# lukecq1231/nats

Measured on NVIDIA H100. Metric: decoder tokens/sec (dim=1000, src=400, |V|=30k) @1/2/4/8 H100 vs Theano CPU, higher is better.
Workload: dtype f32

## Files before the change

nats_b200/csrc/gemm.cu:

```cuda
#include "gemm.cuh"

namespace nats {

namespace {

constexpr int kPad = 4;

template <int BX, int BK, int NT, int PT>
__device__ __forceinline__ void load_kcontig(const float* __restrict__ src, int ld, int x0, int X, int k0,
                                             int kend, bool vec, int tid, float4 (&r)[PT]) {
#pragma unroll
    for (int i = 0; i < PT; ++i) {
        const int v = tid + i * NT;
        float4 val = make_float4(0.f, 0.f, 0.f, 0.f);
        if (v < BX * BK / 4) {
            const int x = v / (BK / 4), kq = (v % (BK / 4)) * 4;
            const int gx = x0 + x, gk = k0 + kq;
            if (gx < X && gk < kend) {
                const float* p = src + (long long)gx * ld + gk;
                if (vec && gk + 3 < kend) {
                    val = __ldg(reinterpret_cast<const float4*>(p));
                } else {
                    val.x = __ldg(p);
                    if (gk + 1 < kend) val.y = __ldg(p + 1);
// ... 210 lines not shown
    else if (ta && !tb) le = launch_pdl(sgemm_kernel<BM, BN, BK, TM, TN, true, false>, grid, block, 0, st, grp);
    else le = launch_pdl(sgemm_kernel<BM, BN, BK, TM, TN, true, true>, grid, block, 0, st, grp);
    NATS_CUDA_OK(le);
    return 0;
}

__global__ void reduce_splits_kernel(const float* __restrict__ part, int nsplit, long long strideP, int M, int N,
                                     int ldp, float* __restrict__ out, int ldo, const float* __restrict__ bias,
                                     int accumulate) {
    pdl_trigger();
    pdl_wait();
    const long long total = (long long)M * N;
    for (long long i = blockIdx.x * (long long)blockDim.x + threadIdx.x; i < total;
         i += (long long)gridDim.x * blockDim.x) {
        const int m = (int)(i / N), n = (int)(i % N);
        float s = sum_strided(part + (long long)m * ldp + n, strideP, nsplit);
        if (bias) s += __ldg(bias + n);
        float* o = out + (long long)m * ldo + n;
        if (accumulate) s += *o;
        *o = s;
    }
}

}

static int g_use_tc = 2;
void gemm_set_tensor_cores(int on) { g_use_tc = on; }
int gemm_get_tensor_cores() { return g_use_tc; }

static bool tc_eligible(const GemmProblem* probs, int count) {
    if (!g_use_tc) return false;
    for (int i = 0; i < count; ++i) {
        const int big = probs[i].M > probs[i].N ? probs[i].M : probs[i].N;
        if (big < 64 || probs[i].K < 32) return false;
    }
    return true;
}


int gemm_launch(cudaStream_t st, const GemmProblem* probs, int count, bool transA, bool transB, int cfg) {
    NATS_REQUIRE(count >= 1 && count <= kGemmMaxGroup, "gemm group size");
    if (tc_eligible(probs, count)) {
        if (g_use_tc >= 2 && tma_gemm_eligible(probs, count)) return tma_gemm_launch(st, probs, count, transA, transB);
        return tc_gemm_launch(st, probs, count, transA, transB);
    }
    GemmGroup grp;
    memset(&grp, 0, sizeof(grp));
    grp.count = count;
    int z = 0, maxM = 0, minN = 1 << 30;
    for (int i = 0; i < count; ++i) {
        grp.p[i] = probs[i];
        NATS_REQUIRE(probs[i].splitk >= 1 && probs[i].splitk <= kGemmMaxSplit && probs[i].batch >= 1, "gemm split/batch");
        NATS_REQUIRE(probs[i].splitk == 1 || !probs[i].accumulate, "split-K cannot accumulate in place");
        NATS_REQUIRE(probs[i].kchunk % 16 == 0 && probs[i].kchunk > 0, "kchunk");
        grp.zstart[i] = z;
        z += probs[i].batch * probs[i].splitk;
        maxM = max(maxM, probs[i].M);
        minN = min(minN, probs[i].N);
    }
    grp.zstart[count] = z;
    for (int i = count; i < kGemmMaxGroup; ++i) grp.zstart[i + 1] = z;
    if (maxM == 0) return 0;
    if (cfg == GEMM_CFG_AUTO) {
        if (maxM <= 32) cfg = GEMM_CFG_SMALLM;
        else if (maxM >= 512 && minN >= 512) cfg = GEMM_CFG_BIG;
        else cfg = GEMM_CFG_MID;
    }
    switch (cfg) {
        case GEMM_CFG_BIG: return launch_cfg<128, 128, 8, 8, 8>(st, grp, transA, transB);
        case GEMM_CFG_MID: return launch_cfg<64, 64, 16, 4, 4>(st, grp, transA, transB);
        case GEMM_CFG_SMALLM: return launch_cfg<32, 128, 16, 4, 4>(st, grp, transA, transB);
        default: break;
    }
    set_error("gemm_launch: bad cfg %d", cfg);
    return 2;
}

int gemm_step_cfg(int M) { return M <= 32 ? GEMM_CFG_SMALLM : GEMM_CFG_MID; }

int gemm_pick_split(const nats_ctx* ctx, int M, int N, int K, int groups) {
    int tiles;
    if (g_use_tc && (M >= 128 || N >= 128) && K >= 32) {
        const int a = M > N ? M : N, b = M > N ? N : M;
        const int bn = b <= 32 ? 32 : 64;
        tiles = cdiv(a, 128) * cdiv(b, bn);
    } else {
        const int bm = (M <= 32) ? 32 : 64, bn = (M <= 32) ? 128 : 64;
        tiles = cdiv(N, bn) * cdiv(M, bm);
    }
    tiles *= (groups > 0 ? groups : 1);
    int s = ctx->num_sms / (tiles > 0 ? tiles : 1);
    s = min(s, K / 64);
    s = min(s, kGemmMaxSplit);
    s = max(s, 1);
    const int chunk = ((cdiv(K, s) + 31) / 32) * 32;
    return max(cdiv(K, chunk), 1);
}

int reduce_splits(cudaStream_t st, const float* part, int nsplit, long long strideP, int M, int N, int ldp,
                  float* out, int ldo, const float* bias, int accumulate) {
    const long long total = (long long)M * N;
    if (total == 0) return 0;
    const int block = 256;
    long long gl = (total + block - 1) / block;
    if (gl > 132LL * 16) gl = 132LL * 16;
    const int grid = (int)gl;
    ProfScope ps(st, K_REDUCE_SPLITS, 0.0, 4.0 * total * (nsplit + 1));
    NATS_CUDA_OK(launch_pdl(reduce_splits_kernel, dim3(grid), dim3(block), 0, st, part, nsplit, strideP, M, N, ldp, out, ldo, bias,
                            accumulate));
    return 0;
}

int gemm_auto(const nats_ctx* ctx, cudaStream_t st, GemmProblem p, bool transA, bool transB, float* scratch,
              long long scratch_floats) {
    if (p.M == 0 || p.N == 0) return 0;
    const bool tc = tc_eligible(&p, 1);
    int cfg = GEMM_CFG_AUTO;
    long long tiles;
    if (tc) {
        const int a = p.M > p.N ? p.M : p.N, b = p.M > p.N ? p.N : p.M;
        const bool swapped = p.M < 128 && p.N > p.M;
        const int nb = swapped ? p.M : p.N, ma = swapped ? p.N : p.M;
        (void)a; (void)b;
        const int bn = nb <= 32 ? 32 : 64;
        tiles = (long long)cdiv(ma, 128) * cdiv(nb, bn) * p.batch;
    } else {
        int bm, bn;
        if (p.M <= 32) { cfg = GEMM_CFG_SMALLM; bm = 32; bn = 128; }
        else if (p.M >= 512 && p.N >= 512) { cfg = GEMM_CFG_BIG; bm = 128; bn = 128; }
        else { cfg = GEMM_CFG_MID; bm = 64; bn = 64; }
        tiles = (long long)cdiv(p.M, bm) * cdiv(p.N, bn) * p.batch;
    }
    int splits = 1;
    if (tc && p.batch == 1 && tiles >= ctx->num_sms && p.K >= 4096 && scratch != nullptr) {
        double best = 1e30;
        for (int s2 = 1; s2 <= 4; ++s2) {
            if ((long long)s2 * p.M * p.N > scratch_floats) break;
            const long long waves = (tiles * s2 + ctx->num_sms - 1) / ctx->num_sms;
            double t = (double)waves * ((double)p.K / s2 / 32.0 * 0.75 + 3.0);
            if (s2 > 1) t += (double)(s2 + 1) * p.M * p.N * 4.0 / 5.0e6;
            if (t < best) { best = t; splits = s2; }
        }
    } else if (p.batch == 1 && tiles < ctx->num_sms && p.K >= 256 && scratch != nullptr) {
        long long want = ((tc ? 1LL : 2LL) * ctx->num_sms + tiles - 1) / tiles;
        if (want > p.K / 128) want = p.K / 128;
        splits = (int)want;
        splits = min(splits, kGemmMaxSplit);
        while (splits > 1 && (long long)splits * p.M * p.N > scratch_floats) --splits;
        if (splits < 1) splits = 1;
    }
    if (splits == 1) return gemm_launch(st, &p, 1, transA, transB, cfg);
    GemmProblem q = p;
    q.C = scratch; q.ldc = p.N; q.bias = nullptr; q.accumulate = 0;
    gemm_set_split(q, splits, (long long)p.M * p.N);
    NATS_TRY(gemm_launch(st, &q, 1, transA, transB, cfg));
    return reduce_splits(st, scratch, splits, (long long)p.M * p.N, p.M, p.N, p.N, p.C, p.ldc, p.bias, p.accumulate);
}

}
```

nats_b200/csrc/tc_common.cuh:

```cuda
#pragma once
#include <cuda.h>

#include "common.cuh"

namespace nats {

bool tma_available();
int tma_map_tile3d(const float* ptr, long long d0, long long d1, long long d2, long long stride1, long long stride2, int b0,
                   int b1, int b2, CUtensorMap* out);

namespace tc {

__device__ __forceinline__ uint32_t smem_u32(const void* p) { return static_cast<uint32_t>(__cvta_generic_to_shared(p)); }
__device__ __forceinline__ void mbar_init(uint64_t* bar, uint32_t count) {
    asm volatile("mbarrier.init.shared::cta.b64 [%0], %1;" ::"r"(smem_u32(bar)), "r"(count) : "memory");
}
__device__ __forceinline__ void mbar_arrive(uint64_t* bar) {
    asm volatile("mbarrier.arrive.shared::cta.b64 _, [%0];" ::"r"(smem_u32(bar)) : "memory");
}
__device__ __forceinline__ void mbar_expect_tx(uint64_t* bar, uint32_t bytes) {
    asm volatile("mbarrier.arrive.expect_tx.shared::cta.b64 _, [%0], %1;" ::"r"(smem_u32(bar)), "r"(bytes) : "memory");
}
__device__ __forceinline__ void mbar_wait(uint64_t* bar, uint32_t parity) {
    uint32_t ok;
    const uint32_t addr = smem_u32(bar);
    do {
        asm volatile(
            "{\n\t.reg .pred p;\n\t"
            "mbarrier.try_wait.parity.shared::cta.b64 p, [%1], %2;\n\t"
            "selp.u32 %0, 1, 0, p;\n\t}"
            : "=r"(ok)
            : "r"(addr), "r"(parity)
            : "memory");
    } while (!ok);
}
__device__ __forceinline__ void tma_load_3d(uint32_t dst, const CUtensorMap* map, uint64_t* bar, int c0, int c1, int c2) {
    asm volatile(
        "cp.async.bulk.tensor.3d.shared::cluster.global.tile.mbarrier::complete_tx::bytes [%0], [%1, {%3, %4, %5}], [%2];"
        ::"r"(dst), "l"(reinterpret_cast<uint64_t>(map)), "r"(smem_u32(bar)), "r"(c0), "r"(c1), "r"(c2)
        : "memory");
}
__device__ __forceinline__ uint64_t desc_sw128(uint32_t saddr) {
    return (uint64_t)((saddr & 0x3FFFF) >> 4) | ((uint64_t)1 << 16) | ((uint64_t)(1024 >> 4) << 32) | ((uint64_t)1 << 62);
}
__device__ __forceinline__ void wgmma_fence() { asm volatile("wgmma.fence.sync.aligned;" ::: "memory"); }
__device__ __forceinline__ void wgmma_commit() { asm volatile("wgmma.commit_group.sync.aligned;" ::: "memory"); }
template <int N>
__device__ __forceinline__ void wgmma_wait() { asm volatile("wgmma.wait_group.sync.aligned %0;" ::"n"(N) : "memory"); }
template <int R>
__device__ __forceinline__ void reg_fence(float (&d)[R]) {
#pragma unroll
    for (int i = 0; i < R; ++i) asm volatile("" : "+f"(d[i])::"memory");
}

__device__ __forceinline__ void wgmma_ss_n32(float (&d)[16], uint64_t da, uint64_t db) {
    asm volatile(
        "{\n\t.reg .pred p;\n\tsetp.ne.b32 p, %18, 0;\n\t"
        "wgmma.mma_async.sync.aligned.m64n32k8.f32.tf32.tf32 {%0,%1,%2,%3,%4,%5,%6,%7,%8,%9,%10,%11,%12,%13,%14,%15}, %16, %17, p, 1, 1;\n\t}"
        : "+f"(d[0]), "+f"(d[1]), "+f"(d[2]), "+f"(d[3]), "+f"(d[4]), "+f"(d[5]), "+f"(d[6]), "+f"(d[7]), "+f"(d[8]), "+f"(d[9]), "+f"(d[10]), "+f"(d[11]), "+f"(d[12]), "+f"(d[13]), "+f"(d[14]), "+f"(d[15])
        : "l"(da), "l"(db), "r"(1));
}
__device__ __forceinline__ void wgmma_ss_n64(float (&d)[32], uint64_t da, uint64_t db) {
    asm volatile(
        "{\n\t.reg .pred p;\n\tsetp.ne.b32 p, %34, 0;\n\t"
        "wgmma.mma_async.sync.aligned.m64n64k8.f32.tf32.tf32 {%0,%1,%2,%3,%4,%5,%6,%7,%8,%9,%10,%11,%12,%13,%14,%15,%16,%17,%18,%19,%20,%21,%22,%23,%24,%25,%26,%27,%28,%29,%30,%31}, %32, %33, p, 1, 1;\n\t}"
        : "+f"(d[0]), "+f"(d[1]), "+f"(d[2]), "+f"(d[3]), "+f"(d[4]), "+f"(d[5]), "+f"(d[6]), "+f"(d[7]), "+f"(d[8]), "+f"(d[9]), "+f"(d[10]), "+f"(d[11]), "+f"(d[12]), "+f"(d[13]), "+f"(d[14]), "+f"(d[15]), "+f"(d[16]), "+f"(d[17]), "+f"(d[18]), "+f"(d[19]), "+f"(d[20]), "+f"(d[21]), "+f"(d[22]), "+f"(d[23]), "+f"(d[24]), "+f"(d[25]), "+f"(d[26]), "+f"(d[27]), "+f"(d[28]), "+f"(d[29]), "+f"(d[30]), "+f"(d[31])
        : "l"(da), "l"(db), "r"(1));
}
__device__ __forceinline__ void wgmma_ss_n128(float (&d)[64], uint64_t da, uint64_t db) {
    asm volatile(
        "{\n\t.reg .pred p;\n\tsetp.ne.b32 p, %66, 0;\n\t"
        "wgmma.mma_async.sync.aligned.m64n128k8.f32.tf32.tf32 {%0,%1,%2,%3,%4,%5,%6,%7,%8,%9,%10,%11,%12,%13,%14,%15,%16,%17,%18,%19,%20,%21,%22,%23,%24,%25,%26,%27,%28,%29,%30,%31,%32,%33,%34,%35,%36,%37,%38,%39,%40,%41,%42,%43,%44,%45,%46,%47,%48,%49,%50,%51,%52,%53,%54,%55,%56,%57,%58,%59,%60,%61,%62,%63}, %64, %65, p, 1, 1;\n\t}"
        : "+f"(d[0]), "+f"(d[1]), "+f"(d[2]), "+f"(d[3]), "+f"(d[4]), "+f"(d[5]), "+f"(d[6]), "+f"(d[7]), "+f"(d[8]), "+f"(d[9]), "+f"(d[10]), "+f"(d[11]), "+f"(d[12]), "+f"(d[13]), "+f"(d[14]), "+f"(d[15]), "+f"(d[16]), "+f"(d[17]), "+f"(d[18]), "+f"(d[19]), "+f"(d[20]), "+f"(d[21]), "+f"(d[22]), "+f"(d[23]), "+f"(d[24]), "+f"(d[25]), "+f"(d[26]), "+f"(d[27]), "+f"(d[28]), "+f"(d[29]), "+f"(d[30]), "+f"(d[31]), "+f"(d[32]), "+f"(d[33]), "+f"(d[34]), "+f"(d[35]), "+f"(d[36]), "+f"(d[37]), "+f"(d[38]), "+f"(d[39]), "+f"(d[40]), "+f"(d[41]), "+f"(d[42]), "+f"(d[43]), "+f"(d[44]), "+f"(d[45]), "+f"(d[46]), "+f"(d[47]), "+f"(d[48]), "+f"(d[49]), "+f"(d[50]), "+f"(d[51]), "+f"(d[52]), "+f"(d[53]), "+f"(d[54]), "+f"(d[55]), "+f"(d[56]), "+f"(d[57]), "+f"(d[58]), "+f"(d[59]), "+f"(d[60]), "+f"(d[61]), "+f"(d[62]), "+f"(d[63])
        : "l"(da), "l"(db), "r"(1));
}
__device__ __forceinline__ void wgmma_rs_n32(float (&d)[16], const uint32_t (&a)[4], uint64_t db) {
    asm volatile(
        "{\n\t.reg .pred p;\n\tsetp.ne.b32 p, %21, 0;\n\t"
        "wgmma.mma_async.sync.aligned.m64n32k8.f32.tf32.tf32 {%0,%1,%2,%3,%4,%5,%6,%7,%8,%9,%10,%11,%12,%13,%14,%15}, {%16,%17,%18,%19}, %20, p, 1, 1;\n\t}"
        : "+f"(d[0]), "+f"(d[1]), "+f"(d[2]), "+f"(d[3]), "+f"(d[4]), "+f"(d[5]), "+f"(d[6]), "+f"(d[7]), "+f"(d[8]), "+f"(d[9]), "+f"(d[10]), "+f"(d[11]), "+f"(d[12]), "+f"(d[13]), "+f"(d[14]), "+f"(d[15])
        : "r"(a[0]), "r"(a[1]), "r"(a[2]), "r"(a[3]), "l"(db), "r"(1));
}
__device__ __forceinline__ void wgmma_rs_n64(float (&d)[32], const uint32_t (&a)[4], uint64_t db) {
    asm volatile(
        "{\n\t.reg .pred p;\n\tsetp.ne.b32 p, %37, 0;\n\t"
        "wgmma.mma_async.sync.aligned.m64n64k8.f32.tf32.tf32 {%0,%1,%2,%3,%4,%5,%6,%7,%8,%9,%10,%11,%12,%13,%14,%15,%16,%17,%18,%19,%20,%21,%22,%23,%24,%25,%26,%27,%28,%29,%30,%31}, {%32,%33,%34,%35}, %36, p, 1, 1;\n\t}"
        : "+f"(d[0]), "+f"(d[1]), "+f"(d[2]), "+f"(d[3]), "+f"(d[4]), "+f"(d[5]), "+f"(d[6]), "+f"(d[7]), "+f"(d[8]), "+f"(d[9]), "+f"(d[10]), "+f"(d[11]), "+f"(d[12]), "+f"(d[13]), "+f"(d[14]), "+f"(d[15]), "+f"(d[16]), "+f"(d[17]), "+f"(d[18]), "+f"(d[19]), "+f"(d[20]), "+f"(d[21]), "+f"(d[22]), "+f"(d[23]), "+f"(d[24]), "+f"(d[25]), "+f"(d[26]), "+f"(d[27]), "+f"(d[28]), "+f"(d[29]), "+f"(d[30]), "+f"(d[31])
        : "r"(a[0]), "r"(a[1]), "r"(a[2]), "r"(a[3]), "l"(db), "r"(1));
}

__device__ __forceinline__ float to_tf32(float x) {
    uint32_t r;
    asm("cvt.rna.tf32.f32 %0, %1;" : "=r"(r) : "f"(x));
    return __uint_as_float(r);
}
__device__ __forceinline__ void st_shared_v4(uint32_t addr, float4 v) {
    asm volatile("st.shared.v4.f32 [%0], {%1,%2,%3,%4};" ::"r"(addr), "f"(v.x), "f"(v.y), "f"(v.z), "f"(v.w) : "memory");
}
__device__ __forceinline__ float resid(float x) { return x - __uint_as_float(__float_as_uint(x) & 0xFFFFE000u); }

template <int R>
__device__ __forceinline__ void gemm_epilogue(const float (&acc0)[R], const float (&acc1)[R], const float (&accx)[R], float* C,
                                              long long c_rs, long long c_cs, int Ma, int Nb, int rb, int cb,
                                              const float* bias_a, const float* bias_n, bool accumulate) {
#pragma unroll
    for (int h = 0; h < 2; ++h) {
        const int i_row = rb + 8 * h;
        if (i_row >= Ma) continue;
        const float ba = bias_a ? __ldg(bias_a + i_row) : 0.f;
        float* crow = C + (long long)i_row * c_rs;
#pragma unroll
        for (int j = 0; j < R / 4; ++j) {
#pragma unroll
            for (int e = 0; e < 2; ++e) {
                const int idx = 4 * j + 2 * h + e;
                const int col = cb + 8 * j + e;
                if (col < Nb) {
                    float o = (acc0[idx] + acc1[idx]) + accx[idx] + ba;
                    if (bias_n) o += __ldg(bias_n + col);
                    float* cp = crow + (long long)col * c_cs;
                    if (accumulate) o += *cp;
                    *cp = o;
                }
            }
        }
    }
}

__device__ __forceinline__ void named_bar_sync(int id, int nthreads) {
    asm volatile("bar.sync %0, %1;" ::"r"(id), "r"(nthreads) : "memory");
}

}
}
```

nats_b200/csrc/tma_gemm.cu:

```cuda
#include <cuda.h>

#include <unordered_map>

#include "gemm.cuh"
#include "ops.cuh"
#include "tc_common.cuh"

namespace nats {

namespace {

typedef CUresult (*EncodeTiledFn)(CUtensorMap*, CUtensorMapDataType, cuuint32_t, void*, const cuuint64_t*,
                                  const cuuint64_t*, const cuuint32_t*, const cuuint32_t*, CUtensorMapInterleave,
                                  CUtensorMapSwizzle, CUtensorMapL2promotion, CUtensorMapFloatOOBfill);
EncodeTiledFn g_encode = nullptr;

struct MapKey {
    const void* ptr; long long inner, outer, ld, batch, bstride; int box_outer; int mn;
    bool operator==(const MapKey& o) const {
        return ptr == o.ptr && inner == o.inner && outer == o.outer && ld == o.ld && batch == o.batch &&
               bstride == o.bstride && box_outer == o.box_outer && mn == o.mn;
    }
};
struct MapKeyHash {
    size_t operator()(const MapKey& k) const {
        size_t h = std::hash<const void*>()(k.ptr);
        auto mix = [&](long long v) { h ^= std::hash<long long>()(v) + 0x9e3779b97f4a7c15ull + (h << 6) + (h >> 2); };
        mix(k.inner); mix(k.outer); mix(k.ld); mix(k.batch); mix(k.bstride); mix(k.box_outer); mix(k.mn);
        return h;
    }
};
std::unordered_map<MapKey, CUtensorMap, MapKeyHash> g_maps;


constexpr int kThreads = 256;
constexpr int kBlockK = 32;
constexpr int kNR = 3;
constexpr int kMaxGroup = 2;

struct TmaProblem {
    float* C;
    const float* bias;
    int Ma, Nb, K;
    long long c_rs, c_cs;
    int batch;
    long long sC;
    int splitk, kchunk;
    long long strideP;
    int accumulate;
    int bias_on_a;
};
struct alignas(64) TmaGroup {
    CUtensorMap mapA[kMaxGroup];
    CUtensorMap mapB[kMaxGroup];
    TmaProblem p[kMaxGroup];
    int zstart[kMaxGroup + 1];
    int count;
};

using namespace tc;

template <int ROWS, bool MN>
__device__ __forceinline__ float raw_at(uint32_t raw, int r, int k) {
    float v;
    asm volatile("ld.shared.f32 %0, [%1];" : "=f"(v) : "r"(raw + 4u * (uint32_t)(MN ? k * ROWS + r : r * 32 + k)));
    return v;
}

template <int ROWS, bool MN>
__device__ __forceinline__ void split_tile(uint32_t raw, uint32_t hi_base, uint32_t lo_base, int klim, int tid) {
    constexpr int kChunks = ROWS * 8;
#pragma unroll
    for (int i = 0; i < (kChunks + kThreads - 1) / kThreads; ++i) {
        const int q = tid + i * kThreads;
        if (q < kChunks) {
            int r, c;
            float4 v;
            if (!MN) {
                r = q >> 3; c = q & 7;
                asm volatile("ld.shared.v4.f32 {%0,%1,%2,%3}, [%4];" : "=f"(v.x), "=f"(v.y), "=f"(v.z), "=f"(v.w)
                             : "r"(raw + 4u * (uint32_t)(r * 32 + 4 * c)));
            } else {
                r = q % ROWS; c = q / ROWS;
                v.x = raw_at<ROWS, true>(raw, r, 4 * c); v.y = raw_at<ROWS, true>(raw, r, 4 * c + 1);
                v.z = raw_at<ROWS, true>(raw, r, 4 * c + 2); v.w = raw_at<ROWS, true>(raw, r, 4 * c + 3);
            }
            if (4 * c >= klim) v.x = 0.f;
            if (4 * c + 1 >= klim) v.y = 0.f;
            if (4 * c + 2 >= klim) v.z = 0.f;
            if (4 * c + 3 >= klim) v.w = 0.f;
            float4 hi, lo;
            hi.x = to_tf32(v.x); hi.y = to_tf32(v.y); hi.z = to_tf32(v.z); hi.w = to_tf32(v.w);
            lo.x = to_tf32(v.x - hi.x); lo.y = to_tf32(v.y - hi.y); lo.z = to_tf32(v.z - hi.z); lo.w = to_tf32(v.w - hi.w);
            const uint32_t off = (uint32_t)(r * 128 + ((c ^ (r & 7)) << 4));
            st_shared_v4(hi_base + off, hi);
            st_shared_v4(lo_base + off, lo);
        }
    }
}

template <int BN>
__device__ __forceinline__ void mma_ss(float (&d)[BN / 2], uint64_t da, uint64_t db) {
    if constexpr (BN == 32) wgmma_ss_n32(d, da, db);
    else wgmma_ss_n64(d, da, db);
}
template <int BN>
__device__ __forceinline__ void mma_rs(float (&d)[BN / 2], const uint32_t (&a)[4], uint64_t db) {
    if constexpr (BN == 32) wgmma_rs_n32(d, a, db);
    else wgmma_rs_n64(d, a, db);
}

template <int BN, bool A_MN, bool B_MN, bool A_REG>
__global__ void __launch_bounds__(kThreads, 1) tma_gemm_kernel(const __grid_constant__ TmaGroup grp) {
    constexpr uint32_t kARaw = 128 * 128, kBRaw = BN * 128;
    constexpr uint32_t kRawStage = kARaw + kBRaw;
    constexpr uint32_t kAHalf = A_REG ? 0 : 128 * 128;
    constexpr uint32_t kSplitStage = 2 * kAHalf + 2 * kBRaw;
    constexpr uint32_t kSplitBase = kNR * kRawStage;
    constexpr int R = BN / 2;
    static_assert(BN == 32 || BN == 64, "BN");

    extern __shared__ __align__(1024) unsigned char smem[];
    __shared__ __align__(8) uint64_t full[kNR];

    int z = blockIdx.z, g = 0;
    if (grp.count > 1 && z >= grp.zstart[1]) g = 1;
    const TmaProblem& P = grp.p[g];
    const CUtensorMap* mapA = &grp.mapA[g];
    const CUtensorMap* mapB = &grp.mapB[g];
    z -= grp.zstart[g];
    const int split = z % P.splitk, batch = z / P.splitk;
    const int m0 = blockIdx.x * 128, n0 = blockIdx.y * BN;
    if (m0 >= P.Ma || n0 >= P.Nb) return;

    const int kbeg = split * P.kchunk;
    const int kend = min(P.K, kbeg + P.kchunk);
    const int nkb = (kend > kbeg) ? (kend - kbeg + kBlockK - 1) / kBlockK : 0;
    const int tid = threadIdx.x, warp = tid >> 5, lane = tid & 31, wg = tid >> 7;
    const uint32_t smem_base = (smem_u32(smem) + 1023u) & ~1023u;

    if (tid == 0) {
        asm volatile("prefetch.tensormap [%0];" ::"l"(mapA) : "memory");
        asm volatile("prefetch.tensormap [%0];" ::"l"(mapB) : "memory");
        for (int s = 0; s < kNR; ++s) mbar_init(&full[s], 1);
        asm volatile("fence.mbarrier_init.release.cluster;" ::: "memory");
    }
    __syncthreads();
    pdl_trigger();
    pdl_wait();

    auto issue = [&](int kb) {
        const int s = kb % kNR;
        const uint32_t raw = smem_base + (uint32_t)s * kRawStage;
        const int k0 = kbeg + kb * kBlockK;
        mbar_expect_tx(&full[s], kRawStage);
        if (A_MN) tma_load_3d(raw, mapA, &full[s], m0, k0, batch);
        else tma_load_3d(raw, mapA, &full[s], k0, m0, batch);
        if (B_MN) tma_load_3d(raw + kARaw, mapB, &full[s], n0, k0, batch);
        else tma_load_3d(raw + kARaw, mapB, &full[s], k0, n0, batch);
    };
    auto split_stage = [&](int kb) {
        mbar_wait(&full[kb % kNR], (uint32_t)((kb / kNR) & 1));
        const uint32_t raw = smem_base + (uint32_t)(kb % kNR) * kRawStage;
        const uint32_t sp = smem_base + kSplitBase + (uint32_t)(kb & 1) * kSplitStage;
        const int klim = kend - (kbeg + kb * kBlockK);
        if (!A_REG) split_tile<128, A_MN>(raw, sp, sp + kAHalf, klim, tid);
        split_tile<BN, B_MN>(raw + kARaw, sp + 2 * kAHalf, sp + 2 * kAHalf + kBRaw, klim, tid);
    };

    float acc0[R], acc1[R], accx[R];
#pragma unroll
    for (int i = 0; i < R; ++i) { acc0[i] = 0.f; acc1[i] = 0.f; accx[i] = 0.f; }
    const int r0 = 64 * wg + 16 * (warp & 3) + (lane >> 2);
    const int q = lane & 3;

    if (nkb > 0) {
        if (tid == 0)
            for (int kb = 0; kb < min(nkb, kNR); ++kb) issue(kb);
        split_stage(0);
    }
    asm volatile("fence.proxy.async.shared::cta;" ::: "memory");
    __syncthreads();
    for (int kb = 0; kb < nkb; ++kb) {
        const uint32_t sp = smem_base + kSplitBase + (uint32_t)(kb & 1) * kSplitStage;
        const uint64_t b_hi = desc_sw128(sp + 2 * kAHalf), b_lo = desc_sw128(sp + 2 * kAHalf + kBRaw);
        if constexpr (A_REG) {
            const uint32_t raw = smem_base + (uint32_t)(kb % kNR) * kRawStage;
            const int klim = kend - (kbeg + kb * kBlockK);
            uint32_t ahi[4][4], alo[4][4];
#pragma unroll
            for (int kk = 0; kk < 4; ++kk) {
#pragma unroll
                for (int f = 0; f < 4; ++f) {
                    const int r = r0 + 8 * (f & 1), k = 8 * kk + q + 4 * (f >> 1);
                    const float x = k < klim ? raw_at<128, A_MN>(raw, r, k) : 0.f;
                    const float h = to_tf32(x);
                    ahi[kk][f] = __float_as_uint(h);
                    alo[kk][f] = __float_as_uint(to_tf32(x - h));
                }
            }
            wgmma_fence();
#pragma unroll
            for (int kk = 0; kk < 4; ++kk) {
                mma_rs<BN>(accx, alo[kk], b_hi + 2 * kk);
                mma_rs<BN>(accx, ahi[kk], b_lo + 2 * kk);
                mma_rs<BN>((kk & 1) ? acc1 : acc0, ahi[kk], b_hi + 2 * kk);
            }
        } else {
            const uint64_t a_hi = desc_sw128(sp + (uint32_t)wg * 8192u), a_lo = desc_sw128(sp + kAHalf + (uint32_t)wg * 8192u);
            wgmma_fence();
#pragma unroll
            for (int kk = 0; kk < 4; ++kk) {
                mma_ss<BN>(accx, a_lo + 2 * kk, b_hi + 2 * kk);
                mma_ss<BN>(accx, a_hi + 2 * kk, b_lo + 2 * kk);
                mma_ss<BN>((kk & 1) ? acc1 : acc0, a_hi + 2 * kk, b_hi + 2 * kk);
            }
        }
        wgmma_commit();
        if (kb + 1 < nkb) split_stage(kb + 1);
        wgmma_wait<0>();
        reg_fence(acc0); reg_fence(acc1); reg_fence(accx);
        asm volatile("fence.proxy.async.shared::cta;" ::: "memory");
        __syncthreads();
        if (tid == 0 && kb + kNR < nkb) issue(kb + kNR);
    }

    const bool add_bias = (P.bias != nullptr) && (split == 0);
    gemm_epilogue(acc0, acc1, accx, P.C + (long long)batch * P.sC + (long long)split * P.strideP, P.c_rs, P.c_cs, P.Ma, P.Nb,
                  m0 + r0, n0 + 2 * q, (add_bias && P.bias_on_a) ? P.bias : nullptr,
                  (add_bias && !P.bias_on_a) ? P.bias : nullptr, P.accumulate != 0);
}

template <int BN, bool A_REG>
constexpr size_t smem_bytes() {
    return (size_t)kNR * (128 * 128 + BN * 128) + 2 * (size_t)(2 * (A_REG ? 0 : 128 * 128) + 2 * BN * 128) + 1024;
}

template <int BN, bool A_REG>
int set_attrs() {
    const int sm = (int)smem_bytes<BN, A_REG>();
    NATS_CUDA_OK(cudaFuncSetAttribute(tma_gemm_kernel<BN, false, false, A_REG>, cudaFuncAttributeMaxDynamicSharedMemorySize, sm));
    NATS_CUDA_OK(cudaFuncSetAttribute(tma_gemm_kernel<BN, false, true, A_REG>, cudaFuncAttributeMaxDynamicSharedMemorySize, sm));
    NATS_CUDA_OK(cudaFuncSetAttribute(tma_gemm_kernel<BN, true, false, A_REG>, cudaFuncAttributeMaxDynamicSharedMemorySize, sm));
    NATS_CUDA_OK(cudaFuncSetAttribute(tma_gemm_kernel<BN, true, true, A_REG>, cudaFuncAttributeMaxDynamicSharedMemorySize, sm));
    return 0;
}

template <int BN, bool A_REG>
int launch_bn(cudaStream_t st, const TmaGroup& grp, bool a_mn, bool b_mn, dim3 grid) {
    const size_t sm = smem_bytes<BN, A_REG>();
    cudaError_t e;
    if (!a_mn && !b_mn) e = launch_pdl(tma_gemm_kernel<BN, false, false, A_REG>, grid, dim3(kThreads), sm, st, grp);
    else if (!a_mn && b_mn) e = launch_pdl(tma_gemm_kernel<BN, false, true, A_REG>, grid, dim3(kThreads), sm, st, grp);
    else if (a_mn && !b_mn) e = launch_pdl(tma_gemm_kernel<BN, true, false, A_REG>, grid, dim3(kThreads), sm, st, grp);
    else e = launch_pdl(tma_gemm_kernel<BN, true, true, A_REG>, grid, dim3(kThreads), sm, st, grp);
    NATS_CUDA_OK(e);
    return 0;
}

int g_ts_mode = 1;

int operand_map(const float* ptr, bool mn, int rows, int K, int ld, int batch, long long bstride, int box_rows, CUtensorMap* out) {
    const long long d0 = mn ? rows : K, d1 = mn ? K : rows;
    return tma_map_tile3d(ptr, d0, d1, batch, ld, batch > 1 ? bstride : d1 * ld, mn ? box_rows : 32, mn ? 32 : box_rows, 1, out);
}

}

bool tma_available() { return g_encode != nullptr; }

int tma_map_tile3d(const float* ptr, long long d0, long long d1, long long d2, long long stride1, long long stride2, int b0,
                   int b1, int b2, CUtensorMap* out) {
    NATS_REQUIRE(g_encode != nullptr, "tensor maps not available");
    MapKey key{ptr, d0, d1, stride1, d2, stride2, b0 * 65536 + b1 * 256 + b2, 2};
    auto it = g_maps.find(key);
    if (it != g_maps.end()) { *out = it->second; return 0; }
    if (g_maps.size() > (1u << 16)) g_maps.clear();
    cuuint64_t gdim[3] = {(cuuint64_t)d0, (cuuint64_t)d1, (cuuint64_t)d2};
    cuuint64_t gstr[2] = {(cuuint64_t)stride1 * 4, (cuuint64_t)stride2 * 4};
    cuuint32_t box[3] = {(cuuint32_t)b0, (cuuint32_t)b1, (cuuint32_t)b2};
    cuuint32_t estr[3] = {1, 1, 1};
    CUtensorMap m;
    const CUresult r = g_encode(&m, CU_TENSOR_MAP_DATA_TYPE_FLOAT32, 3, const_cast<float*>(ptr), gdim, gstr, box, estr,
                                CU_TENSOR_MAP_INTERLEAVE_NONE, CU_TENSOR_MAP_SWIZZLE_NONE, CU_TENSOR_MAP_L2_PROMOTION_L2_256B,
                                CU_TENSOR_MAP_FLOAT_OOB_FILL_NONE);
    if (r != CUDA_SUCCESS) {
        set_error("cuTensorMapEncodeTiled (tile3d) failed (%d): ptr=%p dims=%lld,%lld,%lld strides=%lld,%lld box=%d,%d,%d", (int)r, ptr, d0,
                  d1, d2, stride1, stride2, b0, b1, b2);
        return 1;
    }
    g_maps.emplace(key, m);
    *out = m;
    return 0;
}
void tma_gemm_set_ts(int on) { g_ts_mode = on; }
int tma_gemm_get_ts() { return g_ts_mode; }

int tma_gemm_setup() {
    void* fn = nullptr;
    cudaDriverEntryPointQueryResult q;
    NATS_CUDA_OK(cudaGetDriverEntryPoint("cuTensorMapEncodeTiled", &fn, cudaEnableDefault, &q));
    if (fn == nullptr || q != cudaDriverEntryPointSuccess) {
        set_error("cuTensorMapEncodeTiled not available from the driver");
        return 1;
    }
    g_encode = reinterpret_cast<EncodeTiledFn>(fn);
    NATS_TRY((set_attrs<32, false>()));
    NATS_TRY((set_attrs<64, false>()));
    NATS_TRY((set_attrs<32, true>()));
    NATS_TRY((set_attrs<64, true>()));
    return 0;
}


bool tma_gemm_eligible(const GemmProblem* probs, int count) {
    if (g_encode == nullptr || count > kMaxGroup) return false;
    for (int i = 0; i < count; ++i) {
        const GemmProblem& q = probs[i];
        if ((q.lda & 3) || (q.ldb & 3)) return false;
        if ((reinterpret_cast<uintptr_t>(q.A) & 15) || (reinterpret_cast<uintptr_t>(q.B) & 15)) return false;
        if (q.batch > 1 && ((q.strideA & 3) || (q.strideB & 3))) return false;
        if (q.M < 1 || q.N < 1 || q.K < 1) return false;
    }
    return true;
}

int tma_gemm_launch(cudaStream_t st, const GemmProblem* probs, int count, bool transA, bool transB) {
    NATS_REQUIRE(count >= 1 && count <= kMaxGroup, "tma gemm group size");
    TmaGroup grp;
    memset(&grp, 0, sizeof(grp));
    grp.count = count;
    int maxM = 0, maxN = 0;
    for (int i = 0; i < count; ++i) { maxM = max(maxM, probs[i].M); maxN = max(maxN, probs[i].N); }
    const bool swapped = maxM < 128 && maxN > maxM;
    const int nb_dim = swapped ? maxM : maxN;
    const int BN = nb_dim <= 32 ? 32 : 64;
    const bool skinny = nb_dim <= 64;
    const bool opa_mn = transA, opb_mn = !transB;
    const bool a_mn = swapped ? opb_mn : opa_mn;
    const bool b_mn = swapped ? opa_mn : opb_mn;
    int z = 0, ga = 0, gb = 0;
    double flops = 0.0, bytes = 0.0;
    for (int i = 0; i < count; ++i) {
        const GemmProblem& q = probs[i];
        NATS_REQUIRE(q.splitk >= 1 && q.batch >= 1 && (q.splitk == 1 || !q.accumulate), "tma gemm split/batch");
        TmaProblem& t = grp.p[i];
        CUtensorMap ma, mb;
        NATS_TRY(operand_map(q.A, opa_mn, q.M, q.K, q.lda, q.batch, q.strideA, swapped ? BN : 128, &ma));
        NATS_TRY(operand_map(q.B, opb_mn, q.N, q.K, q.ldb, q.batch, q.strideB, swapped ? 128 : BN, &mb));
        if (!swapped) {
            grp.mapA[i] = ma; grp.mapB[i] = mb;
            t.Ma = q.M; t.Nb = q.N; t.c_rs = q.ldc; t.c_cs = 1; t.bias_on_a = 0;
        } else {
            grp.mapA[i] = mb; grp.mapB[i] = ma;
            t.Ma = q.N; t.Nb = q.M; t.c_rs = 1; t.c_cs = q.ldc; t.bias_on_a = 1;
        }
        t.C = q.C; t.bias = q.bias; t.K = q.K; t.batch = q.batch; t.sC = q.strideC;
        t.splitk = q.splitk;
        t.kchunk = ((q.kchunk + 31) / 32) * 32;
        if (q.splitk > 1) t.kchunk = ((cdiv(q.K, q.splitk) + 31) / 32) * 32;
        if (t.kchunk <= 0) t.kchunk = 32;
        t.strideP = q.strideP; t.accumulate = q.accumulate;
        grp.zstart[i] = z;
        z += q.batch * q.splitk;
        ga = max(ga, cdiv(t.Ma, 128));
        gb = max(gb, cdiv(t.Nb, BN));
        flops += 2.0 * q.M * q.N * q.K * q.batch;
        bytes += 4.0 * q.batch * ((double)q.M * q.K + (double)q.K * q.N + (double)q.M * q.N * q.splitk);
    }
    grp.zstart[count] = z;
    for (int i = count; i < kMaxGroup; ++i) grp.zstart[i + 1] = z;
    if (ga == 0 || gb == 0 || z == 0) return 0;
    dim3 grid(ga, gb, z);
    ProfScope ps(st, skinny ? K_TC_GEMM_SKINNY : K_TC_GEMM, flops, bytes);
    const bool areg = skinny && g_ts_mode;
    if (BN == 32) return areg ? launch_bn<32, true>(st, grp, a_mn, b_mn, grid) : launch_bn<32, false>(st, grp, a_mn, b_mn, grid);
    return areg ? launch_bn<64, true>(st, grp, a_mn, b_mn, grid) : launch_bn<64, false>(st, grp, a_mn, b_mn, grid);
}

}
```

Measured before the change: 34430.

## Add persistent warp-specialized TF32x3 WGMMA kernel with BN 96/112 tiles

Adds a persistent, warp-specialized TMA GEMM kernel for non-skinny problems. One producer warp issues TMA loads, three warps split B into hi/lo TF32 halves, and two consumer warpgroups run register-A WGMMA with n96/n112 shapes, with setmaxnreg rebalancing registers between roles. Tile-count heuristics and the split-K cost model are updated to match the new BN choices. The aim is to overlap loads, operand splitting and MMA and to cut tile waste, at the cost of much more synchronization complexity and new swizzled A-map paths.

```diff
diff --git a/nats_b200/csrc/gemm.cu b/nats_b200/csrc/gemm.cu
--- a/nats_b200/csrc/gemm.cu
+++ b/nats_b200/csrc/gemm.cu
@@ -316,7 +316,7 @@
     int tiles;
     if (g_use_tc && (M >= 128 || N >= 128) && K >= 32) {
         const int a = M > N ? M : N, b = M > N ? N : M;
-        const int bn = b <= 32 ? 32 : 64;
+        const int bn = b <= 32 ? 32 : b <= 64 ? 64 : b <= 112 ? 112 : 96;
         tiles = cdiv(a, 128) * cdiv(b, bn);
     } else {
         const int bm = (M <= 32) ? 32 : 64, bn = (M <= 32) ? 128 : 64;
@@ -356,7 +356,7 @@
         const bool swapped = p.M < 128 && p.N > p.M;
         const int nb = swapped ? p.M : p.N, ma = swapped ? p.N : p.M;
         (void)a; (void)b;
-        const int bn = nb <= 32 ? 32 : 64;
+        const int bn = nb <= 32 ? 32 : nb <= 64 ? 64 : nb <= 112 ? 112 : 96;
         tiles = (long long)cdiv(ma, 128) * cdiv(nb, bn) * p.batch;
     } else {
         int bm, bn;
@@ -371,7 +371,7 @@
         for (int s2 = 1; s2 <= 4; ++s2) {
             if ((long long)s2 * p.M * p.N > scratch_floats) break;
             const long long waves = (tiles * s2 + ctx->num_sms - 1) / ctx->num_sms;
-            double t = (double)waves * ((double)p.K / s2 / 32.0 * 0.75 + 3.0);
+            double t = (double)waves * ((double)p.K / s2 / 32.0 * 1.4 + 3.0);
             if (s2 > 1) t += (double)(s2 + 1) * p.M * p.N * 4.0 / 5.0e6;
             if (t < best) { best = t; splits = s2; }
         }
diff --git a/nats_b200/csrc/tc_common.cuh b/nats_b200/csrc/tc_common.cuh
--- a/nats_b200/csrc/tc_common.cuh
+++ b/nats_b200/csrc/tc_common.cuh
@@ -88,6 +88,24 @@
         : "+f"(d[0]), "+f"(d[1]), "+f"(d[2]), "+f"(d[3]), "+f"(d[4]), "+f"(d[5]), "+f"(d[6]), "+f"(d[7]), "+f"(d[8]), "+f"(d[9]), "+f"(d[10]), "+f"(d[11]), "+f"(d[12]), "+f"(d[13]), "+f"(d[14]), "+f"(d[15]), "+f"(d[16]), "+f"(d[17]), "+f"(d[18]), "+f"(d[19]), "+f"(d[20]), "+f"(d[21]), "+f"(d[22]), "+f"(d[23]), "+f"(d[24]), "+f"(d[25]), "+f"(d[26]), "+f"(d[27]), "+f"(d[28]), "+f"(d[29]), "+f"(d[30]), "+f"(d[31])
         : "r"(a[0]), "r"(a[1]), "r"(a[2]), "r"(a[3]), "l"(db), "r"(1));
 }
+__device__ __forceinline__ void wgmma_rs_n96(float (&d)[48], const uint32_t (&a)[4], uint64_t db) {
+    asm volatile(
+        "{\n\t.reg .pred p;\n\tsetp.ne.b32 p, %53, 0;\n\t"
+        "wgmma.mma_async.sync.aligned.m64n96k8.f32.tf32.tf32 {%0,%1,%2,%3,%4,%5,%6,%7,%8,%9,%10,%11,%12,%13,%14,%15,%16,%17,%18,%19,%20,%21,%22,%23,%24,%25,%26,%27,%28,%29,%30,%31,%32,%33,%34,%35,%36,%37,%38,%39,%40,%41,%42,%43,%44,%45,%46,%47}, {%48,%49,%50,%51}, %52, p, 1, 1;\n\t}"
+        : "+f"(d[0]), "+f"(d[1]), "+f"(d[2]), "+f"(d[3]), "+f"(d[4]), "+f"(d[5]), "+f"(d[6]), "+f"(d[7]), "+f"(d[8]), "+f"(d[9]), "+f"(d[10]), "+f"(d[11]), "+f"(d[12]), "+f"(d[13]), "+f"(d[14]), "+f"(d[15]), "+f"(d[16]), "+f"(d[17]), "+f"(d[18]), "+f"(d[19]), "+f"(d[20]), "+f"(d[21]), "+f"(d[22]), "+f"(d[23]), "+f"(d[24]), "+f"(d[25]), "+f"(d[26]), "+f"(d[27]), "+f"(d[28]), "+f"(d[29]), "+f"(d[30]), "+f"(d[31]), "+f"(d[32]), "+f"(d[33]), "+f"(d[34]), "+f"(d[35]), "+f"(d[36]), "+f"(d[37]), "+f"(d[38]), "+f"(d[39]), "+f"(d[40]), "+f"(d[41]), "+f"(d[42]), "+f"(d[43]), "+f"(d[44]), "+f"(d[45]), "+f"(d[46]), "+f"(d[47])
+        : "r"(a[0]), "r"(a[1]), "r"(a[2]), "r"(a[3]), "l"(db), "r"(1));
+}
+__device__ __forceinline__ void wgmma_rs_n112(float (&d)[56], const uint32_t (&a)[4], uint64_t db) {
+    asm volatile(
+        "{\n\t.reg .pred p;\n\tsetp.ne.b32 p, %61, 0;\n\t"
+        "wgmma.mma_async.sync.aligned.m64n112k8.f32.tf32.tf32 {%0,%1,%2,%3,%4,%5,%6,%7,%8,%9,%10,%11,%12,%13,%14,%15,%16,%17,%18,%19,%20,%21,%22,%23,%24,%25,%26,%27,%28,%29,%30,%31,%32,%33,%34,%35,%36,%37,%38,%39,%40,%41,%42,%43,%44,%45,%46,%47,%48,%49,%50,%51,%52,%53,%54,%55}, {%56,%57,%58,%59}, %60, p, 1, 1;\n\t}"
+        : "+f"(d[0]), "+f"(d[1]), "+f"(d[2]), "+f"(d[3]), "+f"(d[4]), "+f"(d[5]), "+f"(d[6]), "+f"(d[7]), "+f"(d[8]), "+f"(d[9]), "+f"(d[10]), "+f"(d[11]), "+f"(d[12]), "+f"(d[13]), "+f"(d[14]), "+f"(d[15]), "+f"(d[16]), "+f"(d[17]), "+f"(d[18]), "+f"(d[19]), "+f"(d[20]), "+f"(d[21]), "+f"(d[22]), "+f"(d[23]), "+f"(d[24]), "+f"(d[25]), "+f"(d[26]), "+f"(d[27]), "+f"(d[28]), "+f"(d[29]), "+f"(d[30]), "+f"(d[31]), "+f"(d[32]), "+f"(d[33]), "+f"(d[34]), "+f"(d[35]), "+f"(d[36]), "+f"(d[37]), "+f"(d[38]), "+f"(d[39]), "+f"(d[40]), "+f"(d[41]), "+f"(d[42]), "+f"(d[43]), "+f"(d[44]), "+f"(d[45]), "+f"(d[46]), "+f"(d[47]), "+f"(d[48]), "+f"(d[49]), "+f"(d[50]), "+f"(d[51]), "+f"(d[52]), "+f"(d[53]), "+f"(d[54]), "+f"(d[55])
+        : "r"(a[0]), "r"(a[1]), "r"(a[2]), "r"(a[3]), "l"(db), "r"(1));
+}
+template <int N>
+__device__ __forceinline__ void setmaxnreg_dec() { asm volatile("setmaxnreg.dec.sync.aligned.u32 %0;" ::"n"(N)); }
+template <int N>
+__device__ __forceinline__ void setmaxnreg_inc() { asm volatile("setmaxnreg.inc.sync.aligned.u32 %0;" ::"n"(N)); }
 
 __device__ __forceinline__ float to_tf32(float x) {
     uint32_t r;
diff --git a/nats_b200/csrc/tma_gemm.cu b/nats_b200/csrc/tma_gemm.cu
--- a/nats_b200/csrc/tma_gemm.cu
+++ b/nats_b200/csrc/tma_gemm.cu
@@ -55,6 +55,7 @@
     CUtensorMap mapB[kMaxGroup];
     TmaProblem p[kMaxGroup];
     int zstart[kMaxGroup + 1];
+    int istart[kMaxGroup + 1];
     int count;
 };
 
@@ -67,12 +68,12 @@
     return v;
 }
 
-template <int ROWS, bool MN>
+template <int ROWS, bool MN, int NT = kThreads>
 __device__ __forceinline__ void split_tile(uint32_t raw, uint32_t hi_base, uint32_t lo_base, int klim, int tid) {
     constexpr int kChunks = ROWS * 8;
 #pragma unroll
-    for (int i = 0; i < (kChunks + kThreads - 1) / kThreads; ++i) {
-        const int q = tid + i * kThreads;
+    for (int i = 0; i < (kChunks + NT - 1) / NT; ++i) {
+        const int q = tid + i * NT;
         if (q < kChunks) {
             int r, c;
             float4 v;
@@ -231,6 +232,174 @@
                   (add_bias && !P.bias_on_a) ? P.bias : nullptr, P.accumulate != 0);
 }
 
+constexpr int kWsThreads = 384;
+constexpr int kWsNR = 4, kWsNS = 2;
+template <int BN> __host__ __device__ constexpr uint32_t ws_raw() { return 128 * 128 + BN * 128; }
+template <int BN> constexpr size_t ws_smem() { return (size_t)kWsNR * ws_raw<BN>() + (size_t)kWsNS * 2 * BN * 128 + 1024; }
+
+struct WsItem { int g, batch, split, m0, n0, kbeg, kend, nkb; };
+
+template <int BN>
+__device__ __forceinline__ WsItem ws_item(const TmaGroup& grp, int it) {
+    WsItem w;
+    w.g = (grp.count > 1 && it >= grp.istart[1]) ? 1 : 0;
+    const TmaProblem& P = grp.p[w.g];
+    it -= grp.istart[w.g];
+    const int mt = (P.Ma + 127) >> 7, nt = (P.Nb + BN - 1) / BN;
+    w.m0 = (it % mt) * 128; it /= mt;
+    w.n0 = (it % nt) * BN; it /= nt;
+    w.split = it % P.splitk; w.batch = it / P.splitk;
+    w.kbeg = w.split * P.kchunk;
+    w.kend = min(P.K, w.kbeg + P.kchunk);
+    w.nkb = (w.kend > w.kbeg) ? (w.kend - w.kbeg + kBlockK - 1) / kBlockK : 0;
+    return w;
+}
+
+template <bool MN>
+__device__ __forceinline__ float raw_a_sw(uint32_t raw, int r, int k) {
+    const uint32_t off = MN ? (uint32_t)((r >> 5) * 4096 + k * 128 + ((((r & 31) >> 2) ^ (k & 7)) << 4) + (r & 3) * 4)
+                            : (uint32_t)(r * 128 + (((k >> 2) ^ (r & 7)) << 4) + (k & 3) * 4);
+    float v;
+    asm volatile("ld.shared.f32 %0, [%1];" : "=f"(v) : "r"(raw + off));
+    return v;
+}
+template <int N>
+__device__ __forceinline__ void reg_fence_u(uint32_t (&a)[N]) {
+#pragma unroll
+    for (int i = 0; i < N; ++i) asm volatile("" : "+r"(a[i])::"memory");
+}
+
+template <int BN>
+__device__ __forceinline__ void mma_rs_ws(float (&d)[BN / 2], const uint32_t (&a)[4], uint64_t db) {
+    if constexpr (BN == 96) wgmma_rs_n96(d, a, db);
+    else wgmma_rs_n112(d, a, db);
+}
+
+template <int BN, bool A_MN, bool B_MN>
+__global__ void __launch_bounds__(kWsThreads, 1) tma_gemm_kernel_ws(const __grid_constant__ TmaGroup grp, int items) {
+    constexpr uint32_t kRaw = ws_raw<BN>(), kBHalf = BN * 128, kSplit = 2 * kBHalf;
+    constexpr int R = BN / 2;
+    static_assert(BN == 96 || BN == 112, "BN");
+    extern __shared__ __align__(1024) unsigned char smem[];
+    __shared__ __align__(8) uint64_t full[kWsNR], empty[kWsNR], sfull[kWsNS], sempty[kWsNS];
+    const int tid = threadIdx.x, warp = __shfl_sync(0xffffffffu, tid >> 5, 0), lane = tid & 31;
+    const uint32_t smem_base = (smem_u32(smem) + 1023u) & ~1023u;
+    const uint32_t split_base = smem_base + kWsNR * kRaw;
+
+    if (tid == 0) {
+        for (int g = 0; g < grp.count; ++g) {
+            asm volatile("prefetch.tensormap [%0];" ::"l"(&grp.mapA[g]) : "memory");
+            asm volatile("prefetch.tensormap [%0];" ::"l"(&grp.mapB[g]) : "memory");
+        }
+        for (int s = 0; s < kWsNR; ++s) { mbar_init(&full[s], 1); mbar_init(&empty[s], 3 + 8); }
+        for (int s = 0; s < kWsNS; ++s) { mbar_init(&sfull[s], 3); mbar_init(&sempty[s], 2); }
+        asm volatile("fence.mbarrier_init.release.cluster;" ::: "memory");
+    }
+    __syncthreads();
+    pdl_trigger();
+    pdl_wait();
+
+    if (warp < 4) {
+        setmaxnreg_dec<64>();
+        if (warp == 0) {
+            if (lane != 0) return;
+            uint32_t kc = 0;
+            for (int it = blockIdx.x; it < items; it += gridDim.x) {
+                const WsItem w = ws_item<BN>(grp, it);
+                const CUtensorMap* mapA = &grp.mapA[w.g];
+                const CUtensorMap* mapB = &grp.mapB[w.g];
+                for (int kb = 0; kb < w.nkb; ++kb, ++kc) {
+                    const int s = kc % kWsNR;
+                    mbar_wait(&empty[s], ((kc / kWsNR) & 1) ^ 1);
+                    const uint32_t raw = smem_base + (uint32_t)s * kRaw;
+                    const int k0 = w.kbeg + kb * kBlockK;
+                    mbar_expect_tx(&full[s], kRaw);
+                    if (A_MN) {
+#pragma unroll
+                        for (int j = 0; j < 4; ++j) tma_load_3d(raw + 4096u * j, mapA, &full[s], w.m0 + 32 * j, k0, w.batch);
+                    } else {
+                        tma_load_3d(raw, mapA, &full[s], k0, w.m0, w.batch);
+                    }
+                    if (B_MN) tma_load_3d(raw + 128 * 128, mapB, &full[s], w.n0, k0, w.batch);
+                    else tma_load_3d(raw + 128 * 128, mapB, &full[s], k0, w.n0, w.batch);
+                }
+            }
+        } else {
+            const int stid = tid - 32;
+            uint32_t kc = 0;
+            for (int it = blockIdx.x; it < items; it += gridDim.x) {
+                const WsItem w = ws_item<BN>(grp, it);
+                for (int kb = 0; kb < w.nkb; ++kb, ++kc) {
+                    const int s = kc % kWsNR, t = kc % kWsNS;
+                    mbar_wait(&full[s], (kc / kWsNR) & 1);
+                    mbar_wait(&sempty[t], ((kc / kWsNS) & 1) ^ 1);
+                    const uint32_t sp = split_base + (uint32_t)t * kSplit;
+                    split_tile<BN, B_MN, 96>(smem_base + (uint32_t)s * kRaw + 128 * 128, sp, sp + kBHalf,
+                                              w.kend - (w.kbeg + kb * kBlockK), stid);
+                    asm volatile("fence.proxy.async.shared::cta;" ::: "memory");
+                    __syncwarp();
+                    if (lane == 0) { mbar_arrive(&sfull[t]); mbar_arrive(&empty[s]); }
+                }
+            }
+        }
+        return;
+    }
+
+    setmaxnreg_inc<216>();
+    const int ctid = tid - 128, cw = ctid >> 7;
+    const int r0 = 64 * cw + 16 * (warp & 3) + (lane >> 2);
+    const int q = lane & 3;
+    uint32_t kc = 0;
+    for (int it = blockIdx.x; it < items; it += gridDim.x) {
+        const WsItem w = ws_item<BN>(grp, it);
+        const TmaProblem& P = grp.p[w.g];
+        float acc0[R], acc1[R], accx[R];
+#pragma unroll
+        for (int i = 0; i < R; ++i) { acc0[i] = 0.f; acc1[i] = 0.f; accx[i] = 0.f; }
+        uint32_t fa[2][2][4] = {};
+        for (int kb = 0; kb < w.nkb; ++kb, ++kc) {
+            const int s = kc % kWsNR, t = kc % kWsNS;
+            mbar_wait(&full[s], (kc / kWsNR) & 1);
+            mbar_wait(&sfull[t], (kc / kWsNS) & 1);
+            const uint32_t raw = smem_base + (uint32_t)s * kRaw;
+            const uint32_t sp = split_base + (uint32_t)t * kSplit;
+            const uint64_t b_hi = desc_sw128(sp), b_lo = desc_sw128(sp + kBHalf);
+#pragma unroll
+            for (int kk = 0; kk < 4; ++kk) {
+                uint32_t (&ah)[4] = fa[kk & 1][0];
+                uint32_t (&al)[4] = fa[kk & 1][1];
+#pragma unroll
+                for (int f = 0; f < 4; ++f) {
+                    const float x = raw_a_sw<A_MN>(raw, r0 + 8 * (f & 1), 8 * kk + q + 4 * (f >> 1));
+                    const float h = to_tf32(x);
+                    ah[f] = __float_as_uint(h);
+                    al[f] = __float_as_uint(to_tf32(x - h));
+                }
+                if (kk == 3) {
+                    __syncwarp();
+                    if (lane == 0) mbar_arrive(&empty[s]);
+                }
+                wgmma_fence();
+                mma_rs_ws<BN>(accx, al, b_hi + 2 * kk);
+                mma_rs_ws<BN>(accx, ah, b_lo + 2 * kk);
+                mma_rs_ws<BN>((kk & 1) ? acc1 : acc0, ah, b_hi + 2 * kk);
+                wgmma_commit();
+                wgmma_wait<1>();
+                reg_fence_u(fa[(kk + 1) & 1][0]); reg_fence_u(fa[(kk + 1) & 1][1]);
+                if (kk == 0 && kb > 0 && (ctid & 127) == 0) mbar_arrive(&sempty[(kc - 1) % kWsNS]);
+            }
+        }
+        wgmma_wait<0>();
+        reg_fence(acc0); reg_fence(acc1); reg_fence(accx);
+        reg_fence_u(fa[0][0]); reg_fence_u(fa[0][1]); reg_fence_u(fa[1][0]); reg_fence_u(fa[1][1]);
+        if (w.nkb > 0 && (ctid & 127) == 0) mbar_arrive(&sempty[(kc - 1) % kWsNS]);
+        const bool add_bias = (P.bias != nullptr) && (w.split == 0);
+        gemm_epilogue(acc0, acc1, accx, P.C + (long long)w.batch * P.sC + (long long)w.split * P.strideP, P.c_rs, P.c_cs, P.Ma,
+                      P.Nb, w.m0 + r0, w.n0 + 2 * q, (add_bias && P.bias_on_a) ? P.bias : nullptr,
+                      (add_bias && !P.bias_on_a) ? P.bias : nullptr, P.accumulate != 0);
+    }
+}
+
 template <int BN, bool A_REG>
 constexpr size_t smem_bytes() {
     return (size_t)kNR * (128 * 128 + BN * 128) + 2 * (size_t)(2 * (A_REG ? 0 : 128 * 128) + 2 * BN * 128) + 1024;
@@ -258,6 +427,7 @@
     return 0;
 }
 
+int g_num_sms = 0;
 int g_ts_mode = 1;
 
 int operand_map(const float* ptr, bool mn, int rows, int K, int ld, int batch, long long bstride, int box_rows, CUtensorMap* out) {
@@ -269,10 +439,11 @@
 
 bool tma_available() { return g_encode != nullptr; }
 
-int tma_map_tile3d(const float* ptr, long long d0, long long d1, long long d2, long long stride1, long long stride2, int b0,
-                   int b1, int b2, CUtensorMap* out) {
+namespace {
+int encode_tile3d(const float* ptr, long long d0, long long d1, long long d2, long long stride1, long long stride2, int b0, int b1,
+                  int b2, bool swizzle128, CUtensorMap* out) {
     NATS_REQUIRE(g_encode != nullptr, "tensor maps not available");
-    MapKey key{ptr, d0, d1, stride1, d2, stride2, b0 * 65536 + b1 * 256 + b2, 2};
+    MapKey key{ptr, d0, d1, stride1, d2, stride2, b0 * 65536 + b1 * 256 + b2, swizzle128 ? 3 : 2};
     auto it = g_maps.find(key);
     if (it != g_maps.end()) { *out = it->second; return 0; }
     if (g_maps.size() > (1u << 16)) g_maps.clear();
@@ -282,8 +453,8 @@
     cuuint32_t estr[3] = {1, 1, 1};
     CUtensorMap m;
     const CUresult r = g_encode(&m, CU_TENSOR_MAP_DATA_TYPE_FLOAT32, 3, const_cast<float*>(ptr), gdim, gstr, box, estr,
-                                CU_TENSOR_MAP_INTERLEAVE_NONE, CU_TENSOR_MAP_SWIZZLE_NONE, CU_TENSOR_MAP_L2_PROMOTION_L2_256B,
-                                CU_TENSOR_MAP_FLOAT_OOB_FILL_NONE);
+                                CU_TENSOR_MAP_INTERLEAVE_NONE, swizzle128 ? CU_TENSOR_MAP_SWIZZLE_128B : CU_TENSOR_MAP_SWIZZLE_NONE,
+                                CU_TENSOR_MAP_L2_PROMOTION_L2_256B, CU_TENSOR_MAP_FLOAT_OOB_FILL_NONE);
     if (r != CUDA_SUCCESS) {
         set_error("cuTensorMapEncodeTiled (tile3d) failed (%d): ptr=%p dims=%lld,%lld,%lld strides=%lld,%lld box=%d,%d,%d", (int)r, ptr, d0,
                   d1, d2, stride1, stride2, b0, b1, b2);
@@ -292,6 +463,41 @@
     g_maps.emplace(key, m);
     *out = m;
     return 0;
+}
+
+int operand_map_ws_a(const float* ptr, bool mn, int rows, int K, int ld, int batch, long long bstride, CUtensorMap* out) {
+    const long long d0 = mn ? rows : K, d1 = mn ? K : rows;
+    return encode_tile3d(ptr, d0, d1, batch, ld, batch > 1 ? bstride : d1 * ld, 32, mn ? 32 : 128, 1, true, out);
+}
+
+template <int BN>
+int set_attrs_ws() {
+    const int sm = (int)ws_smem<BN>();
+    NATS_CUDA_OK(cudaFuncSetAttribute(tma_gemm_kernel_ws<BN, false, false>, cudaFuncAttributeMaxDynamicSharedMemorySize, sm));
+    NATS_CUDA_OK(cudaFuncSetAttribute(tma_gemm_kernel_ws<BN, false, true>, cudaFuncAttributeMaxDynamicSharedMemorySize, sm));
+    NATS_CUDA_OK(cudaFuncSetAttribute(tma_gemm_kernel_ws<BN, true, false>, cudaFuncAttributeMaxDynamicSharedMemorySize, sm));
+    NATS_CUDA_OK(cudaFuncSetAttribute(tma_gemm_kernel_ws<BN, true, true>, cudaFuncAttributeMaxDynamicSharedMemorySize, sm));
+    return 0;
+}
+
+template <int BN>
+int launch_ws(cudaStream_t st, const TmaGroup& grp, bool a_mn, bool b_mn, int items) {
+    const dim3 grid(min(items, g_num_sms)), block(kWsThreads);
+    const size_t sm = ws_smem<BN>();
+    cudaError_t e;
+    if (!a_mn && !b_mn) e = launch_pdl(tma_gemm_kernel_ws<BN, false, false>, grid, block, sm, st, grp, items);
+    else if (!a_mn && b_mn) e = launch_pdl(tma_gemm_kernel_ws<BN, false, true>, grid, block, sm, st, grp, items);
+    else if (a_mn && !b_mn) e = launch_pdl(tma_gemm_kernel_ws<BN, true, false>, grid, block, sm, st, grp, items);
+    else e = launch_pdl(tma_gemm_kernel_ws<BN, true, true>, grid, block, sm, st, grp, items);
+    NATS_CUDA_OK(e);
+    return 0;
+}
+
+}
+
+int tma_map_tile3d(const float* ptr, long long d0, long long d1, long long d2, long long stride1, long long stride2, int b0,
+                   int b1, int b2, CUtensorMap* out) {
+    return encode_tile3d(ptr, d0, d1, d2, stride1, stride2, b0, b1, b2, false, out);
 }
 void tma_gemm_set_ts(int on) { g_ts_mode = on; }
 int tma_gemm_get_ts() { return g_ts_mode; }
@@ -309,6 +515,11 @@
     NATS_TRY((set_attrs<64, false>()));
     NATS_TRY((set_attrs<32, true>()));
     NATS_TRY((set_attrs<64, true>()));
+    NATS_TRY(set_attrs_ws<96>());
+    NATS_TRY(set_attrs_ws<112>());
+    int dev = 0;
+    NATS_CUDA_OK(cudaGetDevice(&dev));
+    NATS_CUDA_OK(cudaDeviceGetAttribute(&g_num_sms, cudaDevAttrMultiProcessorCount, dev));
     return 0;
 }
 
@@ -334,27 +545,28 @@
     for (int i = 0; i < count; ++i) { maxM = max(maxM, probs[i].M); maxN = max(maxN, probs[i].N); }
     const bool swapped = maxM < 128 && maxN > maxM;
     const int nb_dim = swapped ? maxM : maxN;
-    const int BN = nb_dim <= 32 ? 32 : 64;
     const bool skinny = nb_dim <= 64;
+    const int BN = nb_dim <= 32 ? 32 : nb_dim <= 64 ? 64 : nb_dim <= 112 ? 112 : 96;
     const bool opa_mn = transA, opb_mn = !transB;
     const bool a_mn = swapped ? opb_mn : opa_mn;
     const bool b_mn = swapped ? opa_mn : opb_mn;
-    int z = 0, ga = 0, gb = 0;
+    int z = 0, ga = 0, gb = 0, items = 0;
     double flops = 0.0, bytes = 0.0;
     for (int i = 0; i < count; ++i) {
         const GemmProblem& q = probs[i];
         NATS_REQUIRE(q.splitk >= 1 && q.batch >= 1 && (q.splitk == 1 || !q.accumulate), "tma gemm split/batch");
         TmaProblem& t = grp.p[i];
-        CUtensorMap ma, mb;
-        NATS_TRY(operand_map(q.A, opa_mn, q.M, q.K, q.lda, q.batch, q.strideA, swapped ? BN : 128, &ma));
-        NATS_TRY(operand_map(q.B, opb_mn, q.N, q.K, q.ldb, q.batch, q.strideB, swapped ? 128 : BN, &mb));
-        if (!swapped) {
-            grp.mapA[i] = ma; grp.mapB[i] = mb;
-            t.Ma = q.M; t.Nb = q.N; t.c_rs = q.ldc; t.c_cs = 1; t.bias_on_a = 0;
-        } else {
-            grp.mapA[i] = mb; grp.mapB[i] = ma;
-            t.Ma = q.N; t.Nb = q.M; t.c_rs = 1; t.c_cs = q.ldc; t.bias_on_a = 1;
-        }
+        const float* pa = swapped ? q.B : q.A;
+        const float* pb = swapped ? q.A : q.B;
+        const int rows_a = swapped ? q.N : q.M, rows_b = swapped ? q.M : q.N;
+        const int ld_a = swapped ? q.ldb : q.lda, ld_b = swapped ? q.lda : q.ldb;
+        const long long s_a = swapped ? q.strideB : q.strideA, s_b = swapped ? q.strideA : q.strideB;
+        if (skinny) NATS_TRY(operand_map(pa, a_mn, rows_a, q.K, ld_a, q.batch, s_a, 128, &grp.mapA[i]));
+        else NATS_TRY(operand_map_ws_a(pa, a_mn, rows_a, q.K, ld_a, q.batch, s_a, &grp.mapA[i]));
+        NATS_TRY(operand_map(pb, b_mn, rows_b, q.K, ld_b, q.batch, s_b, BN, &grp.mapB[i]));
+        t.Ma = rows_a; t.Nb = rows_b;
+        if (!swapped) { t.c_rs = q.ldc; t.c_cs = 1; t.bias_on_a = 0; }
+        else { t.c_rs = 1; t.c_cs = q.ldc; t.bias_on_a = 1; }
         t.C = q.C; t.bias = q.bias; t.K = q.K; t.batch = q.batch; t.sC = q.strideC;
         t.splitk = q.splitk;
         t.kchunk = ((q.kchunk + 31) / 32) * 32;
@@ -362,18 +574,23 @@
         if (t.kchunk <= 0) t.kchunk = 32;
         t.strideP = q.strideP; t.accumulate = q.accumulate;
         grp.zstart[i] = z;
+        grp.istart[i] = items;
         z += q.batch * q.splitk;
+        items += q.batch * q.splitk * cdiv(t.Ma, 128) * cdiv(t.Nb, BN);
         ga = max(ga, cdiv(t.Ma, 128));
         gb = max(gb, cdiv(t.Nb, BN));
         flops += 2.0 * q.M * q.N * q.K * q.batch;
         bytes += 4.0 * q.batch * ((double)q.M * q.K + (double)q.K * q.N + (double)q.M * q.N * q.splitk);
     }
     grp.zstart[count] = z;
-    for (int i = count; i < kMaxGroup; ++i) grp.zstart[i + 1] = z;
-    if (ga == 0 || gb == 0 || z == 0) return 0;
+    grp.istart[count] = items;
+    for (int i = count; i < kMaxGroup; ++i) { grp.zstart[i + 1] = z; grp.istart[i + 1] = items; }
+    if (items == 0) return 0;
+    ProfScope ps(st, skinny ? K_TC_GEMM_SKINNY : K_TC_GEMM, flops, bytes);
+    if (BN == 112) return launch_ws<112>(st, grp, a_mn, b_mn, items);
+    if (BN == 96) return launch_ws<96>(st, grp, a_mn, b_mn, items);
     dim3 grid(ga, gb, z);
-    ProfScope ps(st, skinny ? K_TC_GEMM_SKINNY : K_TC_GEMM, flops, bytes);
-    const bool areg = skinny && g_ts_mode;
+    const bool areg = g_ts_mode != 0;
     if (BN == 32) return areg ? launch_bn<32, true>(st, grp, a_mn, b_mn, grid) : launch_bn<32, false>(st, grp, a_mn, b_mn, grid);
     return areg ? launch_bn<64, true>(st, grp, a_mn, b_mn, grid) : launch_bn<64, false>(st, grp, a_mn, b_mn, grid);
 }
```

After: 36360, median of 6. +5.6%, better.
